# jnetter6/RRTQX_3D

Measured on NVIDIA B200. Metric: kd_range_queries_per_s, higher is better.
Workload: dtype f64

## Files before the change

rrtqx_3d_b200/csrc/range_v5.cuh:

```cuda

constexpr int V5_TABPAD = 16;
constexpr int V5_UNIT = 128;
constexpr int V5_RING = 64;
constexpr int V5_U = 4;

__device__ __forceinline__ void sts32(unsigned addr, int v) {
  asm volatile("st.shared.b32 [%0], %1;" ::"r"(addr), "r"(v) : "memory");
}
__device__ __forceinline__ int lds32(unsigned addr) {
  int v;
  asm volatile("ld.shared.b32 %0, [%1];" : "=r"(v) : "r"(addr) : "memory");
  return v;
}
__device__ __forceinline__ unsigned pin_reg(unsigned v) {
  unsigned r;
  asm volatile("mov.u32 %0, %1;" : "=r"(r) : "r"(v));
  return r;
}
__device__ __forceinline__ unsigned long long pk2(float a, float b) {
  unsigned long long r;
  asm("mov.b64 %0, {%1, %2};" : "=l"(r) : "f"(a), "f"(b));
  return r;
}
__device__ __forceinline__ void upk2(unsigned long long r, float &a, float &b) {
  asm("mov.b64 {%0, %1}, %2;" : "=f"(a), "=f"(b) : "l"(r));
}
__device__ __forceinline__ unsigned long long fma2(unsigned long long a, unsigned long long b, unsigned long long c) {
  unsigned long long r;
  asm("fma.rn.f32x2 %0, %1, %2, %3;" : "=l"(r) : "l"(a), "l"(b), "l"(c));
  return r;
}
__device__ __forceinline__ unsigned long long sub2(unsigned long long a, unsigned long long b) {
  unsigned long long r;
  asm("sub.rn.f32x2 %0, %1, %2;" : "=l"(r) : "l"(a), "l"(b));
  return r;
}
__device__ __forceinline__ void sts16(unsigned addr, unsigned v) {
  asm volatile("st.shared.u16 [%0], %1;" ::"r"(addr), "h"((unsigned short)v) : "memory");
}
__device__ __forceinline__ unsigned lds16(unsigned addr) {
  unsigned short v;
  asm volatile("ld.shared.u16 %0, [%1];" : "=h"(v) : "r"(addr) : "memory");
  return v;
}
__device__ __forceinline__ double4 ldg256(const double4 *p) {
  double4 v;
  asm volatile("ld.global.nc.v4.f64 {%0, %1, %2, %3}, [%4];" : "=d"(v.x), "=d"(v.y), "=d"(v.z), "=d"(v.w) : "l"(p));
  return v;
}

__device__ __forceinline__ void v5_st(int32_t *p, int32_t v) { *p = v; }
__device__ __forceinline__ void v5_st(double *p, double v) { *p = v; }

__host__ __device__ __forceinline__ float f32_up(double x) {
#ifdef __CUDA_ARCH__
  return __double2float_ru(x);
#else
  float f = (float)x;
  if ((double)f < x) f = nextafterf(f, INFINITY);
  return f;
#endif
}

__host__ __device__ __forceinline__ void v5_filter(double T, float maxabs_sum, float &Tm, float &M, bool &exact) {
  const float e = maxabs_sum * 6.03e-8f;
  const float Tf = f32_up(T);
  const float sT = sqrtf(Tf);
  Tm = (float)T;
  M = 12.0f * (sT * 1.000001f) * e + 3.9e-6f * Tf;
  exact = !(e * 1024.0f <= sT * 0.999999f) || !(Tf < 1e30f) || !(Tf > 1e-30f);
}

template <int D, bool WRITE>
__device__ __noinline__ int v5_exact_query(const GridView *gp, const double *qptr, double T, double r, int64_t base,
                                           int32_t *__restrict__ out_idx, double *__restrict__ out_dist) {
  const GridView &g = *gp;
  const int lane = lane_id();
  const unsigned lt = lanemask_lt();
  double q[D];
#pragma unroll
  for (int c = 0; c < D; ++c) q[c] = qptr[c];
  int cnt = 0;
  auto visit = [&](bool valid, int node, double px, double py, double pz, double pw) {
    const double s = sqdist<D>(q, px, py, pz, pw);
    const bool hit = valid && (s < T);
    const unsigned m = __ballot_sync(FULL, hit);
    if (WRITE && hit) {
      const int64_t o = base + cnt + __popc(m & lt);
      out_idx[o] = node;
      if (out_dist) out_dist[o] = __dsqrt_rn(s);
    }
    cnt += __popc(m);
  };
  if (g.n_sorted > 0 && r > 0.0) {
    const double r_infl = r * (1.0 + 1e-9);
    const double r2_infl = r_infl * r_infl;
    const int cy0 = cell_of(q[1] - r_infl, g.lo[1], g.inv[1], g.ny);
    const int cy1 = cell_of(q[1] + r_infl, g.lo[1], g.inv[1], g.ny);
    const int cz0 = D >= 3 ? cell_of(q[2] - r_infl, g.lo[2], g.inv[2], g.nz) : 0;
    const int cz1 = D >= 3 ? cell_of(q[2] + r_infl, g.lo[2], g.inv[2], g.nz) : 0;
    const int wy = cy1 - cy0 + 1;
    const int nrows = wy * (cz1 - cz0 + 1);
    for (int rb = 0; rb < nrows; rb += 32) {
      RowSpan sp{0, 0};
      const int row = rb + lane;
      if (row < nrows) sp = row_span<D>(g, q, r2_infl, cy0 + row % wy, cz0 + row / wy);
      const int lim = min(32, nrows - rb);
      for (int t = 0; t < lim; ++t) {
        const int a = __shfl_sync(FULL, sp.start, t);
        const int b = __shfl_sync(FULL, sp.end, t);
        for (int j0 = a; j0 < b; j0 += 32) {
          const int j = j0 + lane;
          const bool v = j < b;
          double4 p = make_double4(0, 0, 0, 0);
          int node = 0;
          if (v) {
            p = g.d4[j];
            node = D <= 3 ? (int)__double_as_longlong(p.w) : g.sperm[j];
          }
          visit(v, node, p.x, p.y, p.z, p.w);
        }
      }
    }
  }
  if (r > 0.0)
    for (int j0 = g.n_sorted; j0 < g.n_total; j0 += 32) {
      const int j = j0 + lane;
      const bool v = j < g.n_total;
      double4 p = make_double4(0, 0, 0, 0);
      if (v) p = g.pos[j];
      visit(v, j, p.x, p.y, p.z, p.w);
    }
  return cnt;
}

template <int D, bool TAIL>
__device__ __forceinline__ void v5_flush(const GridView &g, const double *q, unsigned sbuf_k, unsigned stab, int n, int lane,
                                         int32_t *__restrict__ oi, double *__restrict__ od) {
  constexpr int U = 4;
  auto fetch = [&](unsigned h, int &node, double4 &p) {
    if (!TAIL || !(h & 0x8000u)) {
      const int ent = lds32(stab + 4u * (h >> 3));
      const int slot = (ent >> 4) + (int)(h & 7u);
      p = ldg256(g.d4 + slot);
      node = D <= 3 ? (int)__double_as_longlong(p.w) : g.sperm[slot];
    } else {
      node = g.n_sorted + (int)(h & 0x7fffu);
      p = g.pos[node];
    }
  };
  const int n_full = (n / (32 * U)) * (32 * U);
  for (int h0 = lane; h0 < n_full; h0 += 32 * U) {
    int node[U];
    double4 p[U];
#pragma unroll
    for (int u = 0; u < U; ++u) fetch(lds16(sbuf_k + 2u * (unsigned)(h0 + 32 * u)), node[u], p[u]);
#pragma unroll
    for (int u = 0; u < U; ++u) {
      v5_st(oi + h0 + 32 * u, node[u]);
      if (od) v5_st(od + h0 + 32 * u, __dsqrt_rn(sqdist<D>(q, p[u].x, p[u].y, p[u].z, p[u].w)));
    }
  }
  auto tail = [&](auto rows_tag) {
    constexpr int R = decltype(rows_tag)::value;
    const int h0 = n_full + lane;
    int node[R];
    double4 p[R];
#pragma unroll
    for (int u = 0; u < R; ++u) {
      const int hh = h0 + 32 * u < n ? h0 + 32 * u : 0;
      fetch(lds16(sbuf_k + 2u * (unsigned)hh), node[u], p[u]);
    }
#pragma unroll
    for (int u = 0; u < R; ++u)
      if (h0 + 32 * u < n) {
        v5_st(oi + h0 + 32 * u, node[u]);
        if (od) v5_st(od + h0 + 32 * u, __dsqrt_rn(sqdist<D>(q, p[u].x, p[u].y, p[u].z, p[u].w)));
      }
  };
  const int rem = n - n_full;
  if (rem > 64) tail(std::integral_constant<int, 4>{});
  else if (rem > 32) tail(std::integral_constant<int, 2>{});
  else if (rem > 0) tail(std::integral_constant<int, 1>{});
}

template <int D>
__device__ __noinline__ void v5_flush_tail(const GridView *gp, const double *qs, unsigned sbuf_k, unsigned stab, int n,
                                           int32_t *__restrict__ oi, double *__restrict__ od) {
  double q[D];
#pragma unroll
  for (int c = 0; c < D; ++c) q[c] = qs[c];
  v5_flush<D, true>(*gp, q, sbuf_k, stab, n, lane_id(), oi, od);
}

struct V5Radius {
  float rf, r2f;
  float Tm;
  float cM1, cM0;
  float sum_max;
  bool live;
};
__host__ __device__ __forceinline__ V5Radius v5_radius(double r, double T, bool have) {
  V5Radius R;
  R.live = have && (r > 0.0);
  const double ri = r * (1.0 + 1e-9);
  R.rf = f32_up(ri) * (1.0f + 1e-6f);
  R.r2f = f32_up(ri * ri) * (1.0f + 1e-5f);
  float Tm, M;
  bool ex;
  v5_filter(T, 0.0f, Tm, M, ex);
  const float Tf = f32_up(T), sT = sqrtf(Tf);
  R.Tm = Tm;
  R.cM0 = M;
  R.cM1 = 12.0f * (sT * 1.000001f) * 6.03e-8f * 1.000001f;
  R.sum_max = ex ? -1.0f : sT * 0.999999f * (1.0f / (1024.0f * 6.03e-8f)) * 0.99999f;
  if (!R.live) { R.Tm = -INFINITY; R.r2f = -1.0f; R.cM0 = 0.0f; R.cM1 = 0.0f; R.sum_max = INFINITY; }
  return R;
}

struct V5Params {
  V5Radius RU;
  float invx, invy, invz, celly, cellz;
  unsigned unit;
  int ghost_pairs;
};

__device__ __forceinline__ int clampi_fast(float v, int n) { return min(max(__float2int_rd(v), 0), n - 1); }

__device__ __forceinline__ float sqrt_approx(float x) {
  float y;
  asm("sqrt.approx.f32 %0, %1;" : "=f"(y) : "f"(x));
  return y;
}

template <int D, int NW, int CAP, int TAB, bool UNIFORM>
__global__ void __launch_bounds__(NW * 32, 1)
range_v5_kernel(GridView g_param, V5Params P, const double *__restrict__ queries, const double *__restrict__ qsorted,
                const int32_t *__restrict__ qorder, int64_t nq, double r_uniform, double T_uniform,
                const double *__restrict__ ranges, const double *__restrict__ Tq, int32_t *__restrict__ counts,
                int64_t *__restrict__ offsets, int32_t *__restrict__ out_idx, double *__restrict__ out_dist,
                unsigned long long cap, unsigned long long *__restrict__ cursor, int write_lists) {
  extern __shared__ int s_buf[];
  __shared__ GridView s_g;
  __shared__ unsigned s_ticket;
  __shared__ unsigned s_pub[V5_RING];
  __shared__ long long s_base[V5_RING];
  const GridView &g = g_param;
  if (threadIdx.x == 0) { s_g = g_param; s_ticket = 0; }
  if (threadIdx.x < V5_RING) s_pub[threadIdx.x] = 0;
  __syncthreads();
  const int lane = lane_id(), warp = threadIdx.x >> 5;
  const unsigned lt = lanemask_lt();
  const unsigned s0 = (unsigned)__cvta_generic_to_shared(s_buf);
  const unsigned sbuf = pin_reg(s0 + 2u * (unsigned)(warp * 2 * CAP));
  const unsigned stab = pin_reg(s0 + 2u * (unsigned)(NW * 2 * CAP) + 4u * (unsigned)(warp * (TAB + V5_TABPAD)));
  const float &invx = P.invx, &invy = P.invy, &invz = P.invz, &celly = P.celly, &cellz = P.cellz;
  const float fmaxabs = g.n_sorted > 0 ? *g.fmaxabs : 0.0f;
  const bool has_tail = g.n_total > g.n_sorted;
  const unsigned grp = pin_reg((unsigned)lane >> 3), sub = pin_reg((unsigned)lane & 7u);
  constexpr bool uniform = UNIFORM;

  const int64_t n_pairs = (nq + 1) >> 1;
  for (;;) {
    {
      unsigned tk = 0;
      if (lane == 0) tk = atomicAdd(&s_ticket, 1u);
      tk = __shfl_sync(FULL, tk, 0);
      const unsigned unit = tk / P.unit, off = tk - unit * P.unit, slot = unit % V5_RING;
      long long base = 0;
      if (lane == 0) {
        if (off == 0) {
          base = (long long)atomicAdd(&cursor[1], (unsigned long long)P.unit);
          s_base[slot] = base;
          __threadfence_block();
          atomicExch(&s_pub[slot], unit + 1u);
        } else {
          while (atomicAdd(&s_pub[slot], 0u) != unit + 1u) __nanosleep(32);
          base = *(volatile long long *)&s_base[slot];
        }
      }
      base = __shfl_sync(FULL, base, 0);
      if (base >= n_pairs) break;
      const int64_t qfirst = (base + off) * 2;
      if (qfirst >= nq) continue;
      const bool have1 = qfirst + 1 < nq;
      const int qid0 = qorder[qfirst], qid1 = have1 ? qorder[qfirst + 1] : -1;
      const double *qs0 = qsorted ? qsorted + qfirst * D : queries + (int64_t)qid0 * D;
      const double *qs1 = !have1 ? qs0 : (qsorted ? qs0 + D : queries + (int64_t)qid1 * D);
      V5Radius Rq0, Rq1;
      if (!uniform) {
        Rq0 = v5_radius(ranges[qid0], Tq[qid0], true);
        Rq1 = have1 ? v5_radius(ranges[qid1], Tq[qid1], true) : Rq0;
      }
      const V5Radius &R0 = uniform ? P.RU : Rq0, &R1 = uniform ? P.RU : Rq1;
      auto fp32_query = [&](const double *qs, float (&qf)[4], float &mab) {
        mab = 0.0f;
#pragma unroll
        for (int c = 0; c < 4; ++c) {
          if (c < D) {
            const double v = qs[c];
            qf[c] = __double2float_rn(c < 3 ? __dsub_rn(v, g.lo[c < 3 ? c : 0]) : v);
            mab = fmaxf(mab, fabsf(qf[c]));
          } else {
            qf[c] = 0.0f;
          }
        }
#pragma unroll
        for (int c = 0; c < D; ++c) if (qf[c] != qf[c]) mab = -1.0f;
      };
      auto exactT = [&](int k) { return uniform ? T_uniform : ((k == 0 || !have1) ? Tq[qid0] : Tq[qid1]); };
      auto exactR = [&](int k) { return uniform ? r_uniform : ((k == 0 || !have1) ? ranges[qid0] : ranges[qid1]); };

      int root_extra = 0;
      {
        const double4 p0 = g.pos[0];
        double q0[D], q1[D];
#pragma unroll
        for (int c = 0; c < D; ++c) { q0[c] = qs0[c]; q1[c] = qs1[c]; }
        const double T0 = exactT(0), T1 = exactT(1);
        const double sr0 = sqdist<D>(q0, p0.x, p0.y, p0.z, p0.w), sr1 = sqdist<D>(q1, p0.x, p0.y, p0.z, p0.w);
        if (!(sr0 < T0) && sr0 <= T0 * 1.000001 && __dsqrt_rn(sr0) <= exactR(0)) root_extra |= 1;
        if (have1 && !P.ghost_pairs && !(sr1 < T1) && sr1 <= T1 * 1.000001 && __dsqrt_rn(sr1) <= exactR(1)) root_extra |= 2;
      }
      const bool live0 = R0.live, live1 = R1.live;
      bool exact_path = false;
      int n_ent = 0;
      if (live0 || live1) {
        float qf0[4], qf1[4], mab0, mab1;
        fp32_query(qs0, qf0, mab0);
        fp32_query(qs1, qf1, mab1);
        const bool rows0 = live0 && !(mab0 < 0.0f), rows1 = live1 && !(mab1 < 0.0f);
        exact_path = (rows0 && !(fmaxabs + mab0 <= R0.sum_max)) || (rows1 && !(fmaxabs + mab1 <= R1.sum_max));
        if (!exact_path && g.n_sorted > 0 && (rows0 || rows1)) {
          float ff0[3], ff1[3];
          ff0[0] = qf0[0] * invx; ff0[1] = qf0[1] * invy; ff0[2] = D >= 3 ? qf0[2] * invz : 0.0f;
          ff1[0] = qf1[0] * invx; ff1[1] = qf1[1] * invy; ff1[2] = D >= 3 ? qf1[2] * invz : 0.0f;
          const float ry0 = R0.rf * invy + 1e-3f, ry1 = R1.rf * invy + 1e-3f;
          const float rz0 = R0.rf * invz + 1e-3f, rz1 = R1.rf * invz + 1e-3f;
          int cy0 = 0x7fffffff, cy1 = -1, cz0 = 0, cz1 = 0;
          if (D >= 3) { cz0 = 0x7fffffff; cz1 = -1; }
          if (rows0) {
            cy0 = clampi_fast(ff0[1] - ry0, g.ny); cy1 = clampi_fast(ff0[1] + ry0, g.ny);
            if (D >= 3) { cz0 = clampi_fast(ff0[2] - rz0, g.nz); cz1 = clampi_fast(ff0[2] + rz0, g.nz); }
          }
          if (rows1) {
            cy0 = min(cy0, clampi_fast(ff1[1] - ry1, g.ny)); cy1 = max(cy1, clampi_fast(ff1[1] + ry1, g.ny));
            if (D >= 3) { cz0 = min(cz0, clampi_fast(ff1[2] - rz1, g.nz)); cz1 = max(cz1, clampi_fast(ff1[2] + rz1, g.nz)); }
          }
          const int wy = cy1 - cy0 + 1;
          const int sh = 32 - __clz(wy - 1);
          const int nslots = (cz1 - cz0 + 1) << sh;
          for (int rb = 0; rb < nslots; rb += 32) {
            int sa_ = 0, sb_ = 0;
            const int slot = rb + lane;
            const int ry = slot & ((1 << sh) - 1);
            if (slot < nslots && ry < wy) {
              const int cy = cy0 + ry, cz = cz0 + (slot >> sh);
              const float ylo = cy == 0 ? -INFINITY : (float)cy, yhi = cy == g.ny - 1 ? INFINITY : (float)(cy + 1);
              const float zlo = cz == 0 ? -INFINITY : (float)cz, zhi = cz == g.nz - 1 ? INFINITY : (float)(cz + 1);
              int ca = 0x7fffffff, cb = -1;
              auto span = [&](const float *ff, float r2f) {
                float dy = fmaxf(fmaxf(ylo - ff[1], ff[1] - yhi) * (1.0f - 1e-6f) - 1e-3f, 0.0f) * celly;
                float rem = r2f - dy * dy;
                if (D >= 3) {
                  float dz = fmaxf(fmaxf(zlo - ff[2], ff[2] - zhi) * (1.0f - 1e-6f) - 1e-3f, 0.0f) * cellz;
                  rem -= dz * dz;
                }
                if (rem >= 0.0f) {
                  const float xc = sqrt_approx(rem) * (1.0f + 1e-5f) * invx + 1e-3f;
                  ca = min(ca, clampi_fast(ff[0] - xc, g.nx));
                  cb = max(cb, clampi_fast(ff[0] + xc, g.nx));
                }
              };
              if (rows0) span(ff0, R0.r2f);
              if (rows1) span(ff1, R1.r2f);
              if (cb >= ca) {
                const int rbase = (cz * g.ny + cy) * g.nx;
                sa_ = g.cell_start[rbase + ca];
                sb_ = g.cell_start[rbase + cb + 1];
              }
            }
            const int todo = (sb_ - sa_ + 7) >> 3;
            int incl = todo;
#pragma unroll
            for (int o = 1; o < 32; o <<= 1) {
              const int t = __shfl_up_sync(FULL, incl, o);
              if (lane >= o) incl += t;
            }
            const int sum = __shfl_sync(FULL, incl, 31);
            if (n_ent + sum > TAB) {
              exact_path = true;
              break;
            }
            unsigned ta = stab + 4u * (unsigned)(n_ent + incl - todo);
            for (int i = 0; i < todo; ++i) {
              sts32(ta, (sa_ << 4) | min(8, sb_ - sa_));
              ta += 4u;
              sa_ += 8;
            }
            n_ent += sum;
          }
        }
      }
      int cnt0 = 0, cnt1 = 0;
      bool overflow = false;
      if (exact_path) {
        cnt0 = live0 ? v5_exact_query<D, false>(&s_g, qs0, exactT(0), exactR(0), 0, nullptr, nullptr) : 0;
        cnt1 = (live1 && have1) ? v5_exact_query<D, false>(&s_g, qs1, exactT(1), exactR(1), 0, nullptr, nullptr) : 0;
        overflow = true;
      } else if (live0 || live1) {
        float qf0[4], qf1[4], mab0, mab1;
        fp32_query(qs0, qf0, mab0);
        fp32_query(qs1, qf1, mab1);
        const unsigned long long qx2 = pk2(qf0[0], qf1[0]), qy2 = pk2(qf0[1], qf1[1]);
        const unsigned long long qz2 = pk2(qf0[2], qf1[2]), qw2 = pk2(qf0[3], qf1[3]);
        const unsigned long long nT2 = pk2(-R0.Tm, -R1.Tm);
        const float M = fmaxf(R0.cM1 * (fmaxabs + mab0) + R0.cM0, R1.cM1 * (fmaxabs + mab1) + R1.cM0) * 1.000001f;
        unsigned wp0 = sbuf, wp1 = sbuf + 2u * CAP;
        const unsigned lim0 = sbuf + 2u * (CAP - 32 * V5_U), lim1 = sbuf + 2u * (2 * CAP - 32 * V5_U);

        const unsigned goff = 4u * grp;
        const unsigned hv0 = (grp << 3) | sub;
        int jj[V5_U];
        float4 c[V5_U];
        const int dummy = g.n_sorted + 7;
        auto load_group = [&](unsigned tb) {
          const unsigned taddr = tb + goff;
#pragma unroll
          for (int u = 0; u < V5_U; ++u) {
            const int ent = lds32(taddr + 16u * u);
            jj[u] = sub < (unsigned)(ent & 15) ? (ent >> 4) + (int)sub : dummy;
          }
#pragma unroll
          for (int u = 0; u < V5_U; ++u) {
            c[u] = g.f4[jj[u]];
          }
        };
        auto test_group = [&](auto store_tag, unsigned tb, bool more) {
          constexpr bool STORE = decltype(store_tag)::value;
          const unsigned hv = hv0 + ((tb - stab) << 1);
          float sa[V5_U], sb[V5_U];
          int jc[V5_U];
          float band = INFINITY;
#pragma unroll
          for (int u = 0; u < V5_U; ++u) {
            unsigned long long s2 = sub2(qx2, pk2(c[u].x, c[u].x));
            s2 = fma2(s2, s2, nT2);
            unsigned long long d2 = sub2(qy2, pk2(c[u].y, c[u].y));
            s2 = fma2(d2, d2, s2);
            if (D >= 3) { d2 = sub2(qz2, pk2(c[u].z, c[u].z)); s2 = fma2(d2, d2, s2); }
            if (D >= 4) { d2 = sub2(qw2, pk2(c[u].w, c[u].w)); s2 = fma2(d2, d2, s2); }
            upk2(s2, sa[u], sb[u]);
            band = fminf(band, fminf(fabsf(sa[u]), fabsf(sb[u])));
            jc[u] = jj[u];
          }
          if (more) load_group(tb + 4u * 4 * V5_U);
          if (__any_sync(FULL, band <= M)) {
            double qa[D], qb[D];
#pragma unroll
            for (int cc = 0; cc < D; ++cc) { qa[cc] = qs0[cc]; qb[cc] = qs1[cc]; }
            const double Ta = exactT(0), Tb = exactT(1);
#pragma unroll
            for (int u = 0; u < V5_U; ++u) {
              if (sa[u] < INFINITY || sb[u] < INFINITY) {
                const double4 p = g.d4[jc[u]];
                sa[u] = (live0 && sqdist<D>(qa, p.x, p.y, p.z, p.w) < Ta) ? -INFINITY : INFINITY;
                sb[u] = (live1 && sqdist<D>(qb, p.x, p.y, p.z, p.w) < Tb) ? -INFINITY : INFINITY;
              }
            }
          }
#pragma unroll
          for (int u = 0; u < V5_U; ++u) {
            const bool h0 = sa[u] < M;
            const unsigned m0 = __ballot_sync(FULL, h0);
            if (STORE && h0) sts16(wp0 + 2u * __popc(m0 & lt), hv + 32u * u);
            wp0 += 2u * __popc(m0);
            const bool h1 = sb[u] < M;
            const unsigned m1 = __ballot_sync(FULL, h1);
            if (STORE && h1) sts16(wp1 + 2u * __popc(m1 & lt), hv + 32u * u);
            wp1 += 2u * __popc(m1);
          }
        };
        if (n_ent > 0) {
          if (lane < V5_TABPAD) sts32(stab + 4u * (unsigned)(n_ent + lane), 0);
          __syncwarp();
          unsigned tb = stab;
          const unsigned tend = stab + 4u * (unsigned)n_ent;
          load_group(tb);
          while (tb < tend && wp0 <= lim0 && wp1 <= lim1) {
            const unsigned nb = tb + 4u * 4 * V5_U;
            test_group(std::true_type{}, tb, nb < tend);
            tb = nb;
          }
          if (tb < tend) {
            overflow = true;
            do {
              const unsigned nb = tb + 4u * 4 * V5_U;
              test_group(std::false_type{}, tb, nb < tend);
              tb = nb;
            } while (tb < tend);
          }
          __syncwarp();
        }
        if (has_tail && g.n_total - g.n_sorted > 0x8000) overflow = true;
        if (has_tail) {
          double qa[D], qb[D];
#pragma unroll
          for (int cc = 0; cc < D; ++cc) { qa[cc] = qs0[cc]; qb[cc] = qs1[cc]; }
          const double Ta = exactT(0), Tb = exactT(1);
          for (int j0 = g.n_sorted; j0 < g.n_total; j0 += 32) {
            const int j = j0 + lane;
            const bool v = j < g.n_total;
            double4 p = make_double4(0, 0, 0, 0);
            if (v) p = g.pos[j];
            const bool h0 = v && live0 && (sqdist<D>(qa, p.x, p.y, p.z, p.w) < Ta);
            const bool h1 = v && live1 && (sqdist<D>(qb, p.x, p.y, p.z, p.w) < Tb);
            const unsigned m0 = __ballot_sync(FULL, h0);
            const unsigned o0 = wp0 + 2u * __popc(m0 & lt);
            if (h0 && o0 < sbuf + 2u * CAP) sts16(o0, 0x8000u | (unsigned)((j - g.n_sorted) & 0x7fff));
            wp0 += 2u * __popc(m0);
            const unsigned m1 = __ballot_sync(FULL, h1);
            const unsigned o1 = wp1 + 2u * __popc(m1 & lt);
            if (h1 && o1 < sbuf + 4u * CAP) sts16(o1, 0x8000u | (unsigned)((j - g.n_sorted) & 0x7fff));
            wp1 += 2u * __popc(m1);
          }
        }
        cnt0 = (int)((wp0 - sbuf) >> 1);
        cnt1 = (int)((wp1 - (sbuf + 2u * CAP)) >> 1);
        if (cnt0 > CAP || cnt1 > CAP) overflow = true;
      }
      const bool live1w = live1 && have1;
      if (!have1) cnt1 = 0;

      const int tot0 = cnt0 + (root_extra & 1), tot1 = cnt1 + ((root_extra >> 1) & 1);
      unsigned long long b0 = 0;
      if (lane == 0) b0 = atomicAdd(&cursor[0], (unsigned long long)(tot0 + tot1));
      b0 = __shfl_sync(FULL, b0, 0);
      if (lane == 0) {
        counts[qid0] = tot0;
        offsets[qid0] = (int64_t)b0;
        if (have1) {
          counts[qid1] = tot1;
          offsets[qid1] = (int64_t)(b0 + (unsigned long long)tot0);
        }
      }
      if (!write_lists || b0 + (unsigned long long)(tot0 + tot1) > cap) continue;
      __syncwarp();
      auto emit = [&](int k, const double *qs, int cnt, int64_t base, bool live_k) {
        if (!live_k) return;
        if (overflow) {
          v5_exact_query<D, true>(&s_g, qs, exactT(k), exactR(k), base, out_idx, out_dist);
        } else {
          const unsigned sb_k = sbuf + 2u * (unsigned)(k * CAP);
          if (has_tail) {
            v5_flush_tail<D>(&s_g, qs, sb_k, stab, cnt, out_idx + base, out_dist ? out_dist + base : nullptr);
          } else {
            double q[D];
#pragma unroll
            for (int c = 0; c < D; ++c) q[c] = qs[c];
            v5_flush<D, false>(g, q, sb_k, stab, cnt, lane, out_idx + base, out_dist ? out_dist + base : nullptr);
          }
        }
      };
#pragma unroll 1
      for (int k = 0; k < 2; ++k)
        emit(k, k ? qs1 : qs0, k ? cnt1 : cnt0, (int64_t)b0 + (k ? tot0 : 0), k ? live1w : live0);
      if (root_extra && lane == 0) {
        const double4 p0 = g.pos[0];
        if (root_extra & 1) {
          double q[D];
#pragma unroll
          for (int c = 0; c < D; ++c) q[c] = qs0[c];
          out_idx[b0 + cnt0] = 0;
          if (out_dist) out_dist[b0 + cnt0] = __dsqrt_rn(sqdist<D>(q, p0.x, p0.y, p0.z, p0.w));
        }
        if (root_extra & 2) {
          double q[D];
#pragma unroll
          for (int c = 0; c < D; ++c) q[c] = qs1[c];
          out_idx[b0 + tot0 + cnt1] = 0;
          if (out_dist) out_dist[b0 + tot0 + cnt1] = __dsqrt_rn(sqdist<D>(q, p0.x, p0.y, p0.z, p0.w));
        }
      }
      __syncwarp();
    }
  }
}

template <int D>
__global__ void ghost_expand_kernel(WrapInfo wrap, const double *__restrict__ queries, const double *__restrict__ qsorted,
                                    const int32_t *__restrict__ qorder, int64_t nq, double r,
                                    double *__restrict__ vq, int32_t *__restrict__ vorder) {
  const int64_t j = (int64_t)blockIdx.x * blockDim.x + threadIdx.x;
  if (j >= nq) return;
  const int qid = qorder[j];
  const double *src = qsorted ? qsorted + j * D : queries + (int64_t)qid * D;
  double q[D], gh[D];
#pragma unroll
  for (int k = 0; k < D; ++k) q[k] = src[k];
  const bool used = make_ghost<D>(wrap, q, 1, r, gh);
#pragma unroll
  for (int k = 0; k < D; ++k) {
    vq[(2 * j) * D + k] = q[k];
    vq[(2 * j + 1) * D + k] = used ? gh[k] : __longlong_as_double(0x7ff8000000000000LL);
  }
  vorder[2 * j] = 2 * qid;
  vorder[2 * j + 1] = 2 * qid + 1;
}
__global__ void ghost_merge_kernel(const int32_t *__restrict__ vcounts, const int64_t *__restrict__ voffsets, int64_t nq,
                                   int32_t *__restrict__ counts, int64_t *__restrict__ offsets) {
  const int64_t q = (int64_t)blockIdx.x * blockDim.x + threadIdx.x;
  if (q >= nq) return;
  counts[q] = vcounts[2 * q] + vcounts[2 * q + 1];
  offsets[q] = voffsets[2 * q];
}

template <int D, int NW, int CAP, int TAB>
static void launch_v5(rrtqx_ctx *ctx, const GridView &g, const double *dq, const double *dqs, const int32_t *qorder,
                      int64_t nq, double r, double T, const double *dr, const double *dT, int32_t *counts,
                      int64_t *offsets, int32_t *idx, double *dist, unsigned long long cap, unsigned long long *cursor,
                      int write_lists, int ghost_pairs = 0) {
  const size_t smem = (size_t)NW * (CAP + TAB + V5_TABPAD) * sizeof(int);
  if (ctx->smem_attr_done.insert((const void *)range_v5_kernel<D, NW, CAP, TAB, true>).second) {
    RQ_CUDA(cudaFuncSetAttribute(range_v5_kernel<D, NW, CAP, TAB, true>, cudaFuncAttributeMaxDynamicSharedMemorySize, (int)smem));
    RQ_CUDA(cudaFuncSetAttribute(range_v5_kernel<D, NW, CAP, TAB, false>, cudaFuncAttributeMaxDynamicSharedMemorySize, (int)smem));
  }
  V5Params P;
  P.RU = v5_radius(r, T, true);
  P.invx = (float)g.inv[0]; P.invy = (float)g.inv[1]; P.invz = (float)g.inv[2];
  P.celly = (float)g.cell[1]; P.cellz = (float)g.cell[2];
  P.unit = V5_UNIT;
  P.ghost_pairs = ghost_pairs;
  const int64_t n_units = ((nq + 1) / 2 + P.unit - 1) / P.unit;
  const int blocks = (int)std::max<int64_t>(1, std::min<int64_t>(n_units, (int64_t)ctx->sm_count));
  if (dr)
    range_v5_kernel<D, NW, CAP, TAB, false><<<blocks, NW * 32, smem, ctx->stream>>>(g, P, dq, dqs, qorder, nq, r, T, dr, dT, counts,
                                                                              offsets, idx, dist, cap, cursor, write_lists);
  else
    range_v5_kernel<D, NW, CAP, TAB, true><<<blocks, NW * 32, smem, ctx->stream>>>(g, P, dq, dqs, qorder, nq, r, T, dr, dT, counts,
                                                                             offsets, idx, dist, cap, cursor, write_lists);
  post_launch(ctx);
}

__global__ void thresh_kernel(const double *__restrict__ ranges, int64_t n, double *__restrict__ Tq) {
  int64_t i = (int64_t)blockIdx.x * blockDim.x + threadIdx.x;
  if (i < n) Tq[i] = sqrt_thresh_lt(ranges[i]);
}

template <int D>
static void range_query_fused(rrtqx_tree *t, const double *dq, const double *dr, int64_t nq, double r, uint32_t flags,
                              rrtqx_range_result *res) {
  rrtqx_ctx *ctx = t->ctx;
  cudaStream_t st = ctx->stream;
  const bool count_only = flags & RRTQX_RANGE_COUNT_ONLY;
  const bool want_dist = flags & RRTQX_RANGE_WANT_DIST;
  res->cursor.ensure(4, st);
  {
    PhaseScope p2(ctx, "range_sort");
    sort_queries<D>(t, res, dq, nq);
  }
  const bool ghost = t->wrap.num_wraps == 1;
  const double *kq = dq, *kqs = res->qbins > 0 ? res->qsorted.p : nullptr;
  const int32_t *korder = res->qorder.p;
  int32_t *kcounts = res->counts.p;
  int64_t *koffsets = res->offsets.p;
  int64_t knq = nq;
  if (ghost) {
    res->vq.ensure((size_t)nq * 2 * D, st);
    res->vorder.ensure((size_t)nq * 2, st);
    res->vcounts.ensure((size_t)nq * 2 + 1, st);
    res->voffsets.ensure((size_t)nq * 2 + 1, st);
    ghost_expand_kernel<D><<<div_up(nq, 256), 256, 0, st>>>(t->wrap, dq, kqs, res->qorder.p, nq, r, res->vq.p, res->vorder.p);
    post_launch(ctx);
    kq = nullptr; kqs = res->vq.p; korder = res->vorder.p; kcounts = res->vcounts.p; koffsets = res->voffsets.p; knq = 2 * nq;
  }
  const double T = host_sqrt_thresh_lt(r);
  const double *dT = nullptr;
  if (dr) {
    res->tq.ensure((size_t)nq, st);
    thresh_kernel<<<div_up(nq, 256), 256, 0, st>>>(dr, nq, res->tq.p);
    post_launch(ctx);
    dT = res->tq.p;
  }
  size_t cap = count_only ? 0 : res->idx.cap;
  if (!count_only && want_dist) cap = std::min(cap, res->dist.cap);
  if (!count_only && cap == 0) {
    cap = (size_t)nq * 64;
    res->idx.ensure(cap, st, 0, 1.0);
    if (want_dist) res->dist.ensure(cap, st, 0, 1.0);
    cap = want_dist ? std::min(res->idx.cap, res->dist.cap) : res->idx.cap;
  }
  double k_est = 1e9;
  if (!dr && r > 0.0 && std::isfinite(r)) {
    double vol = 1.0;
    int dims = 0;
    const int nd[3] = {t->nx, t->ny, t->nz};
    for (int c = 0; c < 3; ++c)
      if (nd[c] > 1) { vol *= nd[c] * t->cell[c]; dims++; }
    const double ball = dims == 3 ? 4.18879 * r * r * r : (dims == 2 ? 3.14159 * r * r : 2.0 * r);
    k_est = dims ? 1.15 * (double)t->n * ball / vol : (double)t->n;
  } else if (!dr) {
    k_est = 0.0;
  }
  int variant = k_est <= 576.0 ? 0 : (k_est <= 1280.0 ? 1 : (k_est <= 2048.0 ? 2 : 3));
  if (ctx->tune.fused_variant >= 0) variant = ctx->tune.fused_variant;
  unsigned long long total = 0;
  for (int attempt = 0; attempt < 2; ++attempt) {
    GridView g = t->view();
    RQ_CUDA(cudaMemsetAsync(res->cursor.p, 0, 4 * sizeof(unsigned long long), st));
    {
      PhaseScope p2(ctx, "range_fill");
#define RQ_V5(NW_, CAP_, TAB_)                                                                                       \
  launch_v5<D, NW_, CAP_, TAB_>(ctx, g, kq, kqs, korder, knq, r, T, dr, dT, kcounts, koffsets, res->idx.p, \
                                want_dist ? res->dist.p : nullptr, (unsigned long long)cap, res->cursor.p, count_only ? 0 : 1, ghost ? 1 : 0)
      if (variant == 0) RQ_V5(24, 704, 256);
      else if (variant == 1) RQ_V5(24, 1408, 512);
      else if (variant == 2) RQ_V5(16, 2176, 1024);
      else RQ_V5(8, 4224, 2048);
#undef RQ_V5
    }
    RQ_CUDA(cudaMemcpyAsync(&total, res->cursor.p, sizeof(total), cudaMemcpyDeviceToHost, st));
    RQ_CUDA(cudaStreamSynchronize(st));
    if (count_only || total <= cap) break;
    RQ_REQUIRE(attempt == 0, "internal: range output did not fit after resizing");
    cap = (size_t)total + (size_t)(total / 32) + 1024;
    res->idx.ensure(cap, st, 0, 1.0);
    if (want_dist) res->dist.ensure(cap, st, 0, 1.0);
    cap = want_dist ? std::min(res->idx.cap, res->dist.cap) : res->idx.cap;
  }
  if (ghost) {
    ghost_merge_kernel<<<div_up(nq, 256), 256, 0, st>>>(res->vcounts.p, res->voffsets.p, nq, res->counts.p, res->offsets.p);
    post_launch(ctx);
  }
  res->n_queries = nq;
  res->total = (int64_t)total;
  res->has_lists = !count_only;
  res->has_dist = !count_only && want_dist;
}
```

Before: 359.1 million.

## Skip per-point distance tests for grid cells fully inside both query spheres

For query pairs in 3D, each grid row now computes a conservative x-interval of cells lying entirely inside both queries' radius, using directed-rounding float bounds. Points in those core cells are written as hits straight into both output buffers without distance tests. Only the partial boundary cells go through the usual filtered tests. This cuts per-point distance work for dense neighbourhoods, at the cost of extra scan/shuffle work, a second table region at the end of shared memory, and conservative-bound correctness risk.

```diff
diff --git a/rrtqx_3d_b200/csrc/range_v5.cuh b/rrtqx_3d_b200/csrc/range_v5.cuh
--- a/rrtqx_3d_b200/csrc/range_v5.cuh
+++ b/rrtqx_3d_b200/csrc/range_v5.cuh
@@ -58,6 +58,15 @@
 #else
   float f = (float)x;
   if ((double)f < x) f = nextafterf(f, INFINITY);
+  return f;
+#endif
+}
+__host__ __device__ __forceinline__ float f32_dn(double x) {
+#ifdef __CUDA_ARCH__
+  return __double2float_rd(x);
+#else
+  float f = (float)x;
+  if ((double)f > x) f = nextafterf(f, -INFINITY);
   return f;
 #endif
 }
@@ -198,6 +207,7 @@
   float Tm;
   float cM1, cM0;
   float sum_max;
+  float Ts;
   bool live;
 };
 __host__ __device__ __forceinline__ V5Radius v5_radius(double r, double T, bool have) {
@@ -206,6 +216,7 @@
   const double ri = r * (1.0 + 1e-9);
   R.rf = f32_up(ri) * (1.0f + 1e-6f);
   R.r2f = f32_up(ri * ri) * (1.0f + 1e-5f);
+  R.Ts = f32_dn(T * (1.0 - 1e-5));
   float Tm, M;
   bool ex;
   v5_filter(T, 0.0f, Tm, M, ex);
@@ -221,6 +232,8 @@
 struct V5Params {
   V5Radius RU;
   float invx, invy, invz, celly, cellz;
+  float cyu, czu;
+  float cinvx;
   unsigned unit;
   int ghost_pairs;
 };
@@ -325,6 +338,7 @@
       const bool live0 = R0.live, live1 = R1.live;
       bool exact_path = false;
       int n_ent = 0;
+      int n_core = 0;
       if (live0 || live1) {
         float qf0[4], qf1[4], mab0, mab1;
         fp32_query(qs0, qf0, mab0);
@@ -350,8 +364,10 @@
           const int wy = cy1 - cy0 + 1;
           const int sh = 32 - __clz(wy - 1);
           const int nslots = (cz1 - cz0 + 1) << sh;
+          const bool core_pair = D == 3 && !P.ghost_pairs && rows0 && rows1;
           for (int rb = 0; rb < nslots; rb += 32) {
             int sa_ = 0, sb_ = 0;
+            int ka_ = 0, kb_ = 0;
             const int slot = rb + lane;
             const int ry = slot & ((1 << sh) - 1);
             if (slot < nslots && ry < wy) {
@@ -378,27 +394,59 @@
                 const int rbase = (cz * g.ny + cy) * g.nx;
                 sa_ = g.cell_start[rbase + ca];
                 sb_ = g.cell_start[rbase + cb + 1];
+                ka_ = sb_; kb_ = sb_;
+                if (core_pair && cy > 0 && cy < g.ny - 1 && cz > 0 && cz < g.nz - 1) {
+                  int xa = max(ca, 1), xb = min(cb, g.nx - 2);
+                  auto core = [&](const float *ff, float Ts) {
+                    const float ey = fmaxf(__fsub_ru(ff[1], (float)cy), __fsub_ru((float)(cy + 1), ff[1]));
+                    const float ez = fmaxf(__fsub_ru(ff[2], (float)cz), __fsub_ru((float)(cz + 1), ff[2]));
+                    const float dy = __fmul_ru(__fadd_ru(ey, 1e-3f), P.cyu);
+                    const float dz = __fmul_ru(__fadd_ru(ez, 1e-3f), P.czu);
+                    const float w2 = __fsub_rd(Ts, __fmaf_ru(dy, dy, __fmul_ru(dz, dz)));
+                    if (!(w2 > 0.0f)) { xb = -1; return; }
+                    const float wc = __fmul_rd(sqrt_approx(w2), P.cinvx);
+                    const float sl = __fmaf_ru(fabsf(ff[0]), 1e-6f, 1e-3f);
+                    xa = max(xa, __float2int_ru(__fadd_ru(__fsub_ru(ff[0], wc), sl)));
+                    xb = min(xb, __float2int_rd(__fsub_rd(__fadd_rd(ff[0], wc), sl)) - 1);
+                  };
+                  core(ff0, R0.Ts);
+                  core(ff1, R1.Ts);
+                  if (xb >= xa) {
+                    ka_ = g.cell_start[rbase + xa];
+                    kb_ = g.cell_start[rbase + xb + 1];
+                  }
+                }
               }
             }
-            const int todo = (sb_ - sa_ + 7) >> 3;
-            int incl = todo;
+            const int todo = ((ka_ - sa_ + 7) >> 3) + ((sb_ - kb_ + 7) >> 3), ktodo = (kb_ - ka_ + 7) >> 3;
+            int incl = todo, kincl = ktodo;
 #pragma unroll
             for (int o = 1; o < 32; o <<= 1) {
               const int t = __shfl_up_sync(FULL, incl, o);
-              if (lane >= o) incl += t;
+              const int kt = __shfl_up_sync(FULL, kincl, o);
+              if (lane >= o) { incl += t; kincl += kt; }
             }
-            const int sum = __shfl_sync(FULL, incl, 31);
-            if (n_ent + sum > TAB) {
+            const int sum = __shfl_sync(FULL, incl, 31), ksum = __shfl_sync(FULL, kincl, 31);
+            if (n_ent + sum + n_core + ksum > TAB) {
               exact_path = true;
               break;
             }
             unsigned ta = stab + 4u * (unsigned)(n_ent + incl - todo);
+            int s = sa_, e = ka_;
             for (int i = 0; i < todo; ++i) {
-              sts32(ta, (sa_ << 4) | min(8, sb_ - sa_));
+              if (s >= e) { s = kb_; e = sb_; }
+              sts32(ta, (s << 4) | min(8, e - s));
               ta += 4u;
-              sa_ += 8;
+              s += 8;
+            }
+            ta = stab + 4u * (unsigned)(TAB + V5_TABPAD - n_core - kincl);
+            for (int i = 0; i < ktodo; ++i) {
+              sts32(ta, (ka_ << 4) | min(8, kb_ - ka_));
+              ta += 4u;
+              ka_ += 8;
             }
             n_ent += sum;
+            n_core += ksum;
           }
         }
       }
@@ -481,6 +529,24 @@
             wp1 += 2u * __popc(m1);
           }
         };
+        if (n_core > 0) {
+          const unsigned kend = stab + 4u * (unsigned)(TAB + V5_TABPAD);
+          unsigned nb = 0;
+          for (unsigned tb = kend - 4u * (unsigned)n_core + goff; tb < kend + goff; tb += 16u) {
+            const int ent = tb < kend ? lds32(tb) : 0;
+            const bool h = sub < (unsigned)(ent & 15);
+            const unsigned m = __ballot_sync(FULL, h);
+            if (nb <= lim0 - sbuf) {
+              const unsigned o = nb + 2u * __popc(m & lt), hv = ((tb - stab) << 1) | sub;
+              if (h) { sts16(wp0 + o, hv); sts16(wp1 + o, hv); }
+            } else {
+              overflow = true;
+            }
+            nb += 2u * __popc(m);
+          }
+          wp0 += nb;
+          wp1 += nb;
+        }
         if (n_ent > 0) {
           if (lane < V5_TABPAD) sts32(stab + 4u * (unsigned)(n_ent + lane), 0);
           __syncwarp();
@@ -629,6 +695,8 @@
   P.RU = v5_radius(r, T, true);
   P.invx = (float)g.inv[0]; P.invy = (float)g.inv[1]; P.invz = (float)g.inv[2];
   P.celly = (float)g.cell[1]; P.cellz = (float)g.cell[2];
+  P.cyu = f32_up(g.cell[1] * (1.0 + 2e-6)); P.czu = f32_up(g.cell[2] * (1.0 + 2e-6));
+  P.cinvx = f32_dn(g.inv[0] * (1.0 - 2e-5));
   P.unit = V5_UNIT;
   P.ghost_pairs = ghost_pairs;
   const int64_t n_units = ((nq + 1) / 2 + P.unit - 1) / P.unit;
```

Result: slower. 318.5 million (median of 6 runs) (-11.3%).
